# CristianSimion5/vk-raytracing-engine

Hardware: AMD Instinct MI355X
Metric: Mrays/s (higher is better)
Workload: dtype f32

## Files before the change

### vk-raytracing-engine_amd/csrc/rgen.h

```cpp
#pragma once
#include "device_math.h"
#include "device_scene.h"
#include "shade.h"

struct LaneState
{
  Payload prd;
  f3 curWeight, hitValue, hitValues;
  f3 camOrigin;
  uint32_t px;
  uint32_t lrow;
  int smpl;
  int stage;
};

VKRT_DEV uint32_t globalRow(const TraceParams& P, uint32_t lrow)
{
  if(P.stripRows == 0u)
    return lrow;
  const uint32_t s = lrow / P.stripRows, r = lrow % P.stripRows;
  return (s * P.shardCount + P.shardIndex) * P.stripRows + r;
}

VKRT_DEV bool pixelOfWork(const TraceParams& P, unsigned w, unsigned tileFirst, uint32_t& x, uint32_t& y, uint32_t& lrow)
{
  if(w >= P.tileCount * 64u)
    return false;
  const unsigned tile = tileFirst + (w >> 6), inTile = w & 63u;
  x = (tile % P.tilesX) * 8u + (inTile & 7u);
  lrow = (tile / P.tilesX) * 8u + (inTile >> 3);
  if(x >= P.fullW || lrow >= P.localRows)
    return false;
  y = globalRow(P, lrow);
  return y < P.fullH;
}
VKRT_DEV unsigned pixelSlot(const TraceParams& P, uint32_t x, uint32_t lrow)
{
  return (((lrow >> 3) * P.tilesX + (x >> 3)) << 6) | ((lrow & 7u) << 3) | (x & 7u);
}

VKRT_DEV uint32_t pixelSeed(const TraceParams& P, uint32_t x, uint32_t y)
{
  const uint32_t index = (P.flags & 1u) ? (y * P.fullW + x) : (y * x + x);
  return tea(index, P.seed);
}

VKRT_DEV f3 cameraOrigin(const TraceParams& P)
{
  float origin[4];
  mat4MulVec4(P.viewInverse, 0.0f, 0.0f, 0.0f, 1.0f, origin);
  return mk3(origin[0], origin[1], origin[2]);
}

VKRT_DEV void startSample(const TraceParams& P, LaneState& L)
{
  const float r1 = rnd(L.prd.seed);
  const float r2 = rnd(L.prd.seed);
  const float jx = P.pc.frame == 0 ? 0.5f : r1, jy = P.pc.frame == 0 ? 0.5f : r2;
  const float pcx = (float)L.px + jx, pcy = (float)globalRow(P, L.lrow) + jy;
  const float inU = pcx / (float)P.fullW, inV = pcy / (float)P.fullH;
  const float dx = inU * 2.0f - 1.0f, dy = inV * 2.0f - 1.0f;
  float target[4], direction[4];
  mat4MulVec4(P.projInverse, dx, dy, 1.0f, 1.0f, target);
  const f3 tn = normalize3(mk3(target[0], target[1], target[2]));
  mat4MulVec4(P.viewInverse, tn.x, tn.y, tn.z, 0.0f, direction);
  L.prd.hitValue = mk3(0.0f);
  L.prd.rayOrigin = L.camOrigin;
  L.prd.rayDirection = mk3(direction[0], direction[1], direction[2]);
  L.prd.depth = 0;
  L.prd.weight = mk3(0.0f);
  L.curWeight = mk3(1.0f);
  L.hitValue = mk3(0.0f);
  L.stage = 0;
}

VKRT_DEV void bindPixel(const TraceParams& P, LaneState& L, uint32_t x, uint32_t lrow)
{
  L.px = x; L.lrow = lrow;
  L.prd.isSpecular = false;
  L.prd.lightDist = 0.0f;
  L.prd.shadowRayDir = mk3(0.0f);
  L.camOrigin = cameraOrigin(P);
}

VKRT_DEV void startPixel(const TraceParams& P, LaneState& L, uint32_t x, uint32_t y, uint32_t lrow)
{
  bindPixel(P, L, x, lrow);
  L.prd.seed = pixelSeed(P, x, y);
  L.hitValues = mk3(0.0f);
  L.smpl = 0;
  startSample(P, L);
}

VKRT_DEV void storePixel(const TraceParams& P, const LaneState& L)
{
  const f3 res = L.hitValues / (float)P.pc.samples;
  float4* dst = (float4*)P.image + ((size_t)L.lrow * P.fullW + L.px);
  if(P.pc.frame > 0 && !(P.flags & VKRT_FLAG_STORE_STAGED))
  {
    const float a = 1.0f / (float)(P.pc.frame + 1);
    const float4 old = *dst;
    const f3 m = glsl_mix(mk3(old.x, old.y, old.z), res, a);
    *dst = make_float4(m.x, m.y, m.z, 1.0f);
  }
  else
    *dst = make_float4(res.x, res.y, res.z, 1.0f);
}

VKRT_DEV void blendPixel(float4* dst, float4 staged, int frame)
{
  if(frame > 0)
  {
    const float a = 1.0f / (float)(frame + 1);
    const float4 old = *dst;
    const f3 m = glsl_mix(mk3(old.x, old.y, old.z), mk3(staged.x, staged.y, staged.z), a);
    *dst = make_float4(m.x, m.y, m.z, 1.0f);
  }
  else
    *dst = make_float4(staged.x, staged.y, staged.z, 1.0f);
}

VKRT_DEV bool afterClosestRay(const TraceParams& P, LaneState& L, const RayHit& hit, const uint4 ts, f3 rayDir, ShadeStats& st)
{
  if(hit.slot >= 0)
    closestHitShader(P.sc, P.pc, hit, ts, rayDir, L.prd, st);
  else
    missShader(P.pc, L.prd);
  if(!L.prd.isSpecular && L.prd.depth != 100u)
  {
    L.stage = 1;
    return true;
  }
  return false;
}

VKRT_DEV void segmentTerms(const Payload& prd, f3 curWeight, f3& contrib, f3& nextWeight)
{
  const f3 q = prd.hitValue * curWeight;
  contrib = mk3(glsl_min(q.x, 10.0f), glsl_min(q.y, 10.0f), glsl_min(q.z, 10.0f));
  nextWeight = curWeight * prd.weight;
}

enum SegmentStep
{
  SEG_PIXEL_DONE = 0,
  SEG_CONTINUE = 1,
  SEG_SAMPLE_END = 2
};
VKRT_DEV SegmentStep stepSegment(const TraceParams& P, LaneState& L, bool shadowHit, f3 contrib, f3 nextWeight)
{
  L.stage = 0;
  if(!shadowHit)
    L.hitValue = L.hitValue + contrib;
  L.curWeight = nextWeight;
  L.prd.depth++;
  if(L.prd.depth < (uint32_t)P.pc.depth)
    return SEG_CONTINUE;
  L.hitValues = L.hitValues + L.hitValue;
  L.smpl++;
  if(L.smpl < P.pc.samples)
    return SEG_SAMPLE_END;
  storePixel(P, L);
  return SEG_PIXEL_DONE;
}

VKRT_DEV bool advanceSegment(const TraceParams& P, LaneState& L, bool shadowHit, f3 contrib, f3 nextWeight)
{
  const SegmentStep step = stepSegment(P, L, shadowHit, contrib, nextWeight);
  if(step == SEG_SAMPLE_END)
    startSample(P, L);
  return step != SEG_PIXEL_DONE;
}

VKRT_DEV bool accumulateAndAdvance(const TraceParams& P, LaneState& L, bool shadowHit)
{
  f3 contrib, nextWeight;
  segmentTerms(L.prd, L.curWeight, contrib, nextWeight);
  return advanceSegment(P, L, shadowHit, contrib, nextWeight);
}
```

### vk-raytracing-engine_amd/csrc/shade.h

```cpp
#pragma once
#include "device_math.h"
#include "device_scene.h"
#include "texel.h"
#include "traverse.h"

struct Payload
{
  f3 hitValue;
  uint32_t seed;
  uint32_t depth;
  f3 rayOrigin, rayDirection, weight;
  bool isSpecular;
  float lightDist;
  f3 shadowRayDir;
};

struct ShadeStats
{
  unsigned hits, diffuse, taps;
  const float* lut;
};

VKRT_DEV const float* ldsTexelLut(const DevScene& sc, float* lds512)
{
// ... 61 lines not shown
  st.taps++;
  f4 r;
  if(sc.textureCount == 0u || texIndex < 0 || texIndex >= (int)sc.textureCount)
  {
    r.x = r.y = r.z = r.w = 1.0f;
    return r;
  }
  DevTexture tx = sc.textures[texIndex];
  const uint32_t levels = tx.srgb >> 8;
  if(!g.on || levels <= 1u)
    return sampleTexLevel(sc, tx, nullptr, 0u, u, v, st.lut);
  const uint32_t* levelOffsets = sc.texMips + (size_t)texIndex * VKRT_MAX_MIPS;
  const float fw = (float)tx.width, fh = (float)tx.height;
  const float mxu = g.dudx * fw, mxv = g.dvdx * fh, myu = g.dudy * fw, myv = g.dvdy * fh;
  const float rx2 = mxu * mxu + mxv * mxv, ry2 = myu * myu + myv * myv;
  const bool majorX = rx2 >= ry2;
  const float rmax = sqrtf(majorX ? rx2 : ry2), rmin = sqrtf(majorX ? ry2 : rx2);
  float eta = 1.0f;
  if(rmin > 0.0f)
    eta = glsl_min(rmax / rmin, 4.0f);
  else if(rmax > 0.0f)
    eta = 4.0f;
  if(!(eta >= 1.0f))
    eta = 1.0f;
  const int N = (int)ceilf(eta);
  const float scale = rmax / eta;
  float lambda = 0.0f;
  if(scale > 1.0f && scale < 3.0e38f)
    lambda = lodLog2(scale);
  else if(!(scale <= 1.0f))
    lambda = (float)(levels - 1u);
  lambda = glsl_clamp(lambda, 0.0f, (float)(levels - 1u));
  const float fl = floorf(lambda), delta = lambda - fl;
  const uint32_t hi = (uint32_t)fl, lo = hi + 1u < levels ? hi + 1u : levels - 1u;
  const float du = majorX ? g.dudx : g.dudy, dv = majorX ? g.dvdx : g.dvdy;
  r.x = r.y = r.z = r.w = 0.0f;
  for(int i = 1; i <= N; i++)
  {
    const float o = (float)i / (float)(N + 1) - 0.5f;
    float tu = u + o * du, tv = v + o * dv;
    if(!(fabsf(tu) < 1.0e9f) || !(fabsf(tv) < 1.0e9f))
    {
      tu = u;
      tv = v;
    }
    const f4 a = sampleTexLevel(sc, tx, levelOffsets, hi, tu, tv, st.lut), b = sampleTexLevel(sc, tx, levelOffsets, lo, tu, tv, st.lut);
    r.x = r.x + (a.x * (1.0f - delta) + b.x * delta);
    r.y = r.y + (a.y * (1.0f - delta) + b.y * delta);
    r.z = r.z + (a.z * (1.0f - delta) + b.z * delta);
    r.w = r.w + (a.w * (1.0f - delta) + b.w * delta);
  }
  const float inv = 1.0f / (float)N;
  r.x = r.x * inv; r.y = r.y * inv; r.z = r.z * inv; r.w = r.w * inv;
  return r;
}

VKRT_DEV f3 pbrGetBaseColor(const DevScene& sc, const GltfPBRMaterial& mat, float tu, float tv, const TexGrad& g, ShadeStats& st)
{
  f3 color = mk3(mat.pbrBaseColorFactor[0], mat.pbrBaseColorFactor[1], mat.pbrBaseColorFactor[2]);
  if(mat.pbrBaseColorTexture > -1)
  {
    const f4 t = sampleTex(sc, mat.pbrBaseColorTexture, tu, tv, g, st);
    color = color * mk3(t.x, t.y, t.z);
  }
  return color;
}
VKRT_DEV void pbrGetMetallicRoughness(const DevScene& sc, const GltfPBRMaterial& mat, float tu, float tv, const TexGrad& g,
                                      float& metallic, float& roughness, ShadeStats& st)
{
  metallic = mat.metallicFactor;
  roughness = mat.roughnessFactor;
  if(mat.metallicRoughnessTexture > -1)
  {
    const f4 t = sampleTex(sc, mat.metallicRoughnessTexture, tu, tv, g, st);
    roughness *= t.y;
    metallic *= t.z;
  }
}
VKRT_DEV float getNDF_GGXTR(f3 N, f3 H, float alpha)
{
  float a2 = alpha * alpha;
  float NH = dot3(N, H);
  if(NH <= 0.0f)
    return 0.0f;
  float NH2 = NH * NH;
  float d = NH2 * (a2 - 1.0f) + 1.0f;
  return a2 * VKRT_INV_PI / (d * d + 1e-4f);
}
VKRT_DEV float getG_SchlickGGX(float NV, float k) { return NV / (NV * (1.0f - k) + k); }
VKRT_DEV float getG_Smith(f3 N, f3 V, f3 L, float k)
{
  float NV = fabsf(dot3(N, V));
  float NL = fabsf(dot3(N, L));
  return getG_SchlickGGX(NV, k) * getG_SchlickGGX(NL, k);
}
VKRT_DEV f3 getF_Schlick(f3 H, f3 V, f3 F0)
{
  return F0 + (mk3(1.0f) - F0) * vk_pow5(1.0f - fabsf(dot3(H, V)));
}
VKRT_DEV f3 getSpecularBRDF_Cook_Torrance(f3 N, f3 H, f3 V, f3 L, f3 F0, float roughness)
{
  float alpha = roughness * roughness;
  float k = (roughness + 1.0f) * (roughness + 1.0f) / 8.0f;
  float D = getNDF_GGXTR(N, H, alpha);
  float G = getG_Smith(N, V, L, k);
  f3 F = getF_Schlick(H, V, F0);
  float down = 4.0f * fabsf(dot3(V, N)) * fabsf(dot3(L, N)) + 1e-4f;
  return D * F * G / down;
}
VKRT_DEV f3 getSpecularBRDF_over_pdf_Cook_Torrance(f3 N, f3 H, f3 V, f3 L, f3 F0, float roughness, float ratio)
{
  float k = (roughness + 1.0f) * (roughness + 1.0f) / 8.0f;
  float pdf = (1.0f - ratio) * dot3(N, H) / (4.0f * dot3(L, H) + 1e-4f);
  float G = getG_Smith(N, V, L, k);
  f3 F = getF_Schlick(H, V, F0);
  float down = 4.0f * fabsf(dot3(V, N)) * fabsf(dot3(L, N)) + 1e-4f;
  return (F * G / down) / pdf;
}
VKRT_DEV f3 computePBR_BRDF(f3 N, f3 V, f3 L, f3 H, f3 baseColor, float metalness, float roughness)
{
  f3 F0 = mk3(0.04f);
  F0 = glsl_mix(F0, baseColor, metalness);
  f3 F = getF_Schlick(H, V, F0);
  f3 f_cook_torrance = getSpecularBRDF_Cook_Torrance(N, H, V, L, F0, roughness);
  f3 kD = mk3(1.0f) - F;
  kD = kD * (1.0f - metalness);
  f3 f_lambert = baseColor * VKRT_INV_PI;
  f3 diffuse = kD * f_lambert;
  return diffuse + f_cook_torrance;
}
VKRT_DEV f3 directLight(const GltfLight& light, f3 P, f3 N, f3 V, f3 baseColor, float metalness, float roughness, unsigned retap,
                        f3& Li, float& cosTheta, ShadeStats& st)
{
  Li = mk3(0.0f);
  cosTheta = 0.0f;
  if(light.type == 0)
  {
    f3 Ldir = mk3(light.position[0], light.position[1], light.position[2]) - P;
    float d = length3(Ldir);
    f3 L = Ldir / d;
    f3 H = normalize3(L + V);
    float attenuation = d * d;
    Li = mk3(light.color[0], light.color[1], light.color[2]) * light.intensity / attenuation;
    cosTheta = glsl_max(dot3(L, N), 0.0f);
    if(cosTheta > 0.0f)
    {
      st.taps += retap;
      return computePBR_BRDF(N, V, L, H, baseColor, metalness, roughness);
    }
  }
  return mk3(0.0f);
}

VKRT_DEV f3 xformPoint(const DevInstance& in, f3 p)
{
  f3 r;
  r.x = ((in.o2w[0] * p.x + in.o2w[1] * p.y) + in.o2w[2] * p.z) + in.o2w[3];
  r.y = ((in.o2w[4] * p.x + in.o2w[5] * p.y) + in.o2w[6] * p.z) + in.o2w[7];
  r.z = ((in.o2w[8] * p.x + in.o2w[9] * p.y) + in.o2w[10] * p.z) + in.o2w[11];
  return r;
}
VKRT_DEV f3 xformNormal(const DevInstance& in, f3 n)
{
  f3 r;
  r.x = (n.x * in.w2o[0] + n.y * in.w2o[3]) + n.z * in.w2o[6];
  r.y = (n.x * in.w2o[1] + n.y * in.w2o[4]) + n.z * in.w2o[7];
  r.z = (n.x * in.w2o[2] + n.y * in.w2o[5]) + n.z * in.w2o[8];
  return r;
}

struct HitMid
{
  f3 worldPos, N, tangent, binormal, V, baseColor, emittance;
  float metalU, roughU;
  unsigned retap;
};

VKRT_DEV void closestHitFront(const DevScene& sc, const RayHit& hit, const uint32_t instId, const uint4 ts, f3 worldRayDir, const Payload& prd,
                              ShadeStats& st, HitMid& mid)
{
  st.hits++;
  const uint32_t i0 = ts.x, i1 = ts.y, i2 = ts.z, matIndex = ts.w;
  const f3 b = mk3(1.0f - hit.u - hit.v, hit.u, hit.v);

  const BufView vPN = bufView(sc.vertexPN), vMat = bufView(sc.shadeMaterials), vInst = bufView(sc.instances);
  const float4 a0 = bufLoad4(vPN, VKRT_VERTEX_BYTES * i0), b0 = bufLoad4(vPN, VKRT_VERTEX_BYTES * i0 + 16u), tq0 = bufLoad4(vPN, VKRT_VERTEX_BYTES * i0 + 32u);
  const float4 a1 = bufLoad4(vPN, VKRT_VERTEX_BYTES * i1), b1 = bufLoad4(vPN, VKRT_VERTEX_BYTES * i1 + 16u), tq1 = bufLoad4(vPN, VKRT_VERTEX_BYTES * i1 + 32u);
  const float4 a2 = bufLoad4(vPN, VKRT_VERTEX_BYTES * i2), b2 = bufLoad4(vPN, VKRT_VERTEX_BYTES * i2 + 16u), tq2 = bufLoad4(vPN, VKRT_VERTEX_BYTES * i2 + 32u);
  const uint32_t mo = 64u * matIndex;
  const float4 m0 = bufLoad4(vMat, mo), m1 = bufLoad4(vMat, mo + 16u), ref01 = bufLoad4(vMat, mo + 32u), ref23 = bufLoad4(vMat, mo + 48u);
  const uint32_t dimB = __float_as_uint(ref01.x), baseB = __float_as_uint(ref01.y), dimM = __float_as_uint(ref01.z), baseM = __float_as_uint(ref01.w);
  const uint32_t dimN = __float_as_uint(ref23.x), baseN = __float_as_uint(ref23.y), dimE = __float_as_uint(ref23.z), baseE = __float_as_uint(ref23.w);
  DevInstance in;
  {
    const uint32_t io = 96u * instId;
    const float4 q0 = bufLoad4(vInst, io), q1 = bufLoad4(vInst, io + 16u), q2 = bufLoad4(vInst, io + 32u), q3 = bufLoad4(vInst, io + 48u), q4 = bufLoad4(vInst, io + 64u),
                 q5 = bufLoad4(vInst, io + 80u);
    in.o2w[0] = q0.x; in.o2w[1] = q0.y; in.o2w[2] = q0.z; in.o2w[3] = q0.w; in.o2w[4] = q1.x; in.o2w[5] = q1.y; in.o2w[6] = q1.z; in.o2w[7] = q1.w;
    in.o2w[8] = q2.x; in.o2w[9] = q2.y; in.o2w[10] = q2.z; in.o2w[11] = q2.w;
    in.w2o[0] = q3.x; in.w2o[1] = q3.y; in.w2o[2] = q3.z; in.w2o[3] = q3.w; in.w2o[4] = q4.x; in.w2o[5] = q4.y; in.w2o[6] = q4.z; in.w2o[7] = q4.w;
    in.w2o[8] = q5.x; in.primMesh = __float_as_int(q5.y); in.vis = 0u; in.pad = 0;
  }
  GltfPBRMaterial mat;
  mat.pbrBaseColorFactor[0] = m0.x; mat.pbrBaseColorFactor[1] = m0.y; mat.pbrBaseColorFactor[2] = m0.z; mat.pbrBaseColorFactor[3] = 1.0f;
  mat.metallicFactor = m0.w; mat.roughnessFactor = m1.x;
  mat.emissiveFactor[0] = m1.y; mat.emissiveFactor[1] = m1.z; mat.emissiveFactor[2] = m1.w;
  mat.pbrBaseColorTexture = (dimB & 0x8000u) ? 0 : -1; mat.metallicRoughnessTexture = (dimM & 0x8000u) ? 0 : -1;
  mat.normalTexture = (dimN & 0x8000u) ? 0 : -1; mat.emissiveTexture = (dimE & 0x8000u) ? 0 : -1;
  const float tu = (b0.z * b.x + b1.z * b.y) + b2.z * b.z;
  const float tv = (b0.w * b.x + b1.w * b.y) + b2.w * b.z;

  const bool emits = prd.depth == 0 || prd.isSpecular;
  const bool wantE = emits && mat.emissiveTexture > -1, wantN = mat.normalTexture > -1;
  const bool wantB = mat.pbrBaseColorTexture > -1, wantM = mat.metallicRoughnessTexture > -1;
  st.taps += (wantE ? 1u : 0u) + (wantN ? 1u : 0u) + (wantB ? 1u : 0u) + (wantM ? 1u : 0u);
  TexTap tE, tN, tB, tM;
  uint32_t e00 = 0u, e10 = 0u, e01 = 0u, e11 = 0u, n00 = 0u, n10 = 0u, n01 = 0u, n11 = 0u;
  uint32_t c00 = 0u, c10 = 0u, c01 = 0u, c11 = 0u, r00 = 0u, r10 = 0u, r01 = 0u, r11 = 0u;
  const bool pool = sc.texQuads != nullptr;
  const BufView gather = bufView(pool ? (const void*)sc.texQuads : (const void*)sc.texels);
#define VKRT_TAP(dim, base, want, tap, a, b, c, d)                                                                                     \
  if(__ballot(want) != 0ull)                                                                                                           \
  {                                                                                                                                    \
    const uint32_t w_ = ((dim) & 0x7fffu) + 1u, h_ = (((dim) >> 16) & 0x7fffu) + 1u;                                                   \
    const bool live_ = (want) && ((dim) >> 31) != 0u;                                                                                  \
    int x0_, y0_;                                                                                                                      \
    texFootprintOrigin(w_, h_, ((base) >> 31) != 0u, ((dim) >> 31) != 0u, tu, tv, tap, x0_, y0_);                                      \
    if(pool)                                                                                                                           \
    {                                                                                                                                  \
      const uint32_t rec_ = live_ ? ((uint32_t)y0_ * w_ + (uint32_t)x0_) + ((base) & 0x7fffffffu) : 0u;                                 \
      const float4 v_ = bufLoad4(gather, 16u * rec_);                                                                                  \
      a = __float_as_uint(v_.x); b = __float_as_uint(v_.y); c = __float_as_uint(v_.z); d = __float_as_uint(v_.w);                      \
    }                                                                                                                                  \
    else                                                                                                                               \
    {                                                                                                                                  \
      texFootprintTexels((base) & 0x7fffffffu, w_, h_, live_, x0_, y0_, tap);                                                          \
      a = bufLoad1(gather, 4u * tap.i00); b = bufLoad1(gather, 4u * tap.i10);                                                          \
      c = bufLoad1(gather, 4u * tap.i01); d = bufLoad1(gather, 4u * tap.i11);                                                          \
    }                                                                                                                                  \
  }
  VKRT_TAP(dimE, baseE, wantE, tE, e00, e10, e01, e11)
  VKRT_TAP(dimN, baseN, wantN, tN, n00, n10, n01, n11)
  VKRT_TAP(dimB, baseB, wantB, tB, c00, c10, c01, c11)
  VKRT_TAP(dimM, baseM, wantM, tM, r00, r10, r01, r11)
#undef VKRT_TAP

  const f3 pos = mk3(a0.x, a0.y, a0.z) * b.x + mk3(a1.x, a1.y, a1.z) * b.y + mk3(a2.x, a2.y, a2.z) * b.z;
  const f3 worldPos = xformPoint(in, pos);
  const f3 nrm = normalize3(mk3(a0.w, b0.x, b0.y) * b.x + mk3(a1.w, b1.x, b1.y) * b.y + mk3(a2.w, b2.x, b2.y) * b.z);
  const f3 worldNrm = normalize3(xformNormal(in, nrm));
  const f3 tag = normalize3(mk3(tq0.x, tq0.y, tq0.z) * b.x + mk3(tq1.x, tq1.y, tq1.z) * b.y + mk3(tq2.x, tq2.y, tq2.z) * b.z);
  f3 worldTag = normalize3(xformNormal(in, tag));
  worldTag = normalize3(worldTag - dot3(worldTag, worldNrm) * worldNrm);
  const f3 worldBin = tq0.w * cross3(worldNrm, worldTag);

  f3 emittance = mk3(0.0f);
  if(emits)
  {
    emittance = mk3(mat.emissiveFactor[0], mat.emissiveFactor[1], mat.emissiveFactor[2]);
    if(wantE)
    {
      const f4 t = texBlend(st.lut, tE, e00, e10, e01, e11);
      emittance = emittance * mk3(t.x, t.y, t.z);
    }
  }
  f3 tangent = worldTag, binormal = worldBin;
  f3 texNormal = worldNrm;
  if(wantN)
  {
    const f4 t = texBlend(st.lut, tN, n00, n10, n01, n11);
    texNormal = normalize3(mk3(t.x, t.y, t.z) * 2.0f - mk3(1.0f));
    texNormal = normalize3(tangent * texNormal.x + binormal * texNormal.y + worldNrm * texNormal.z);
    createCoordinateSystem(texNormal, tangent, binormal);
  }
  f3 baseColor = mk3(mat.pbrBaseColorFactor[0], mat.pbrBaseColorFactor[1], mat.pbrBaseColorFactor[2]);
  if(wantB)
  {
    const f4 t = texBlend(st.lut, tB, c00, c10, c01, c11);
    baseColor = baseColor * mk3(t.x, t.y, t.z);
  }
  float metalness = mat.metallicFactor, roughness = mat.roughnessFactor;
  if(wantM)
  {
    const f4 t = texBlend(st.lut, tM, r00, r10, r01, r11);
    roughness *= t.y;
    metalness *= t.z;
  }

  mid.worldPos = worldPos; mid.N = texNormal; mid.tangent = tangent; mid.binormal = binormal;
  mid.V = normalize3(-worldRayDir);
  mid.baseColor = baseColor; mid.emittance = emittance;
  mid.metalU = metalness; mid.roughU = roughness;
  mid.retap = (mat.pbrBaseColorTexture > -1 ? 1u : 0u) + (mat.metallicRoughnessTexture > -1 ? 1u : 0u);
}

VKRT_DEV bool closestHitLobe(const HitMid& mid, Payload& prd)
{
  const float ratio = 0.5f * (1.0f - mid.metalU);
  const float r1 = rnd(prd.seed);
  return r1 < ratio;
}

VKRT_DEV void closestHitTail(const DevScene& sc, const PushConstantRay& pc, const HitMid& mid, const bool diffuse, Payload& prd, ShadeStats& st)
{
  const f3 worldPos = mid.worldPos, texNormal = mid.N, tangent = mid.tangent, binormal = mid.binormal, V = mid.V, N = mid.N;
  const f3 baseColor = mid.baseColor;
  f3 emittance = mid.emittance;
  const float metalU = mid.metalU, roughU = mid.roughU;
  const unsigned retap = mid.retap;
  const float ratio = 0.5f * (1.0f - metalU);
  const float roughness = glsl_clamp(roughU, 0.01f, 0.99f);
  const float metalness = glsl_clamp(metalU, 0.01f, 0.99f);
  const f3 rayOrigin = worldPos;
  f3 rayDirection;
  float pdf;
  f3 BRDF;
  if(diffuse)
  {
    st.diffuse++;
    prd.isSpecular = false;
    const int random_index = (int)(rnd(prd.seed) * (float)pc.lightsCount);
    const float4* lq = (const float4*)&sc.lights[random_index];
    const float4 l0 = lq[0], l1 = lq[1];
    GltfLight light;
    light.position[0] = l0.x; light.position[1] = l0.y; light.position[2] = l0.z;
    light.color[0] = l0.w; light.color[1] = l1.x; light.color[2] = l1.y;
    light.intensity = l1.z; light.type = __float_as_int(l1.w);
    const f3 lightDir = mk3(light.position[0], light.position[1], light.position[2]) - worldPos;
    const float lightDistance = length3(lightDir);
    const f3 L = normalize3(lightDir);
    prd.lightDist = lightDistance;
    prd.shadowRayDir = L;
    if(dot3(L, texNormal) <= 0)
      emittance = emittance + mk3(0.0f);
    else
    {
      f3 Li;
      float cosTheta;
      const f3 brdf = directLight(light, worldPos, texNormal, V, baseColor, metalU, roughU, retap, Li, cosTheta, st);
      emittance = emittance + (float)pc.lightsCount * brdf * Li * cosTheta;
    }
    rayDirection = normalize3(samplingHemisphere(prd.seed, tangent, binormal, texNormal));
    pdf = ratio * dot3(rayDirection, texNormal) * VKRT_INV_PI;
    BRDF = (1.0f - metalness) * baseColor * VKRT_INV_PI;
  }
  else
  {
    prd.isSpecular = true;
    const float alpha = roughness * roughness;
    const f3 h = samplingNDF_GGXTR(prd.seed, alpha * alpha);
    const f3 H = normalize3(tangent * h.x + binormal * h.y + texNormal * h.z);
    const f3 L = normalize3(glsl_reflect(-V, H));
    rayDirection = L;
    f3 F0 = mk3(0.04f);
    F0 = glsl_mix(F0, baseColor, metalness);
    pdf = 1.0f;
    BRDF = getSpecularBRDF_over_pdf_Cook_Torrance(N, H, V, L, F0, roughness, ratio);
  }
  const float cosTheta = dot3(rayDirection, texNormal);
  prd.rayOrigin = rayOrigin;
  prd.rayDirection = rayDirection;
  prd.hitValue = emittance;
  prd.weight = BRDF * cosTheta / pdf;
}

VKRT_DEV void closestHitShaderInst(const DevScene& sc, const PushConstantRay& pc, const RayHit& hit, const uint32_t instId, const uint4 ts,
                                   f3 worldRayDir, Payload& prd, ShadeStats& st)
{
  HitMid mid;
  closestHitFront(sc, hit, instId, ts, worldRayDir, prd, st, mid);
  const bool diffuse = closestHitLobe(mid, prd);
  closestHitTail(sc, pc, mid, diffuse, prd, st);
}

VKRT_DEV void closestHitShader(const DevScene& sc, const PushConstantRay& pc, const RayHit& hit, const uint4 ts, f3 worldRayDir, Payload& prd,
                               ShadeStats& st)
{
  const uint32_t instId = (uint32_t)__float_as_int(sc.tris[hit.slot * VKRT_TRI_QUADS + 2].z);
  closestHitShaderInst(sc, pc, hit, instId, ts, worldRayDir, prd, st);
}
VKRT_DEV void closestHitShader(const DevScene& sc, const PushConstantRay& pc, const RayHit& hit, f3 worldRayDir, Payload& prd, ShadeStats& st)
{
  closestHitShader(sc, pc, hit, sc.triShade[hit.slot], worldRayDir, prd, st);
}

VKRT_DEV void missShader(const PushConstantRay& pc, Payload& prd)
{
  if(prd.depth == 0)
    prd.hitValue = mk3(pc.clearColor[0], pc.clearColor[1], pc.clearColor[2]) * 0.8f;
  else
    prd.hitValue = mk3(0.01f);
  prd.depth = 100;
}

VKRT_DEV void mat4MulVec4(const float* M, float v0, float v1, float v2, float v3, float* out)
{
#pragma unroll
  for(int i = 0; i < 4; i++)
    out[i] = ((M[0 + i] * v0 + M[4 + i] * v1) + M[8 + i] * v2) + M[12 + i] * v3;
}
```

### vk-raytracing-engine_amd/csrc/wavefront.hip

```cpp
#include <hip/hip_runtime.h>
#include <algorithm>
#include <cstdlib>
#include <cstring>

#include "device_math.h"
#include "device_scene.h"
#include "kernels.h"
#include "rgen.h"
#include "hybrid_gi.h"
#include "shade.h"
#include "traverse.h"
#include "traverse_wide.h"
#include "traverse_share.h"

#define WF_BLOCK 256
#define VKRT_FLAG_COUNT_WORK 2u

#include "wf_streams.h"

VKRT_DEV unsigned packFlags(const LaneState& L)
{
  return (L.prd.depth & 0xffu) | (((unsigned)L.smpl & 0xffffu) << 8) | ((L.prd.isSpecular ? 1u : 0u) << 25);
}

VKRT_DEV void loadCommon(const TraceParams& P, const WfBuffers& B, int parity, int type, unsigned i, LaneState& L)
{
  const float4 s0 = wfLoad(rec(B, parity, type, WF_S0, i)), s1 = wfLoad(rec(B, parity, type, WF_S1, i)), s2 = wfLoad(rec(B, parity, type, WF_S2, i));
  const unsigned flags = __float_as_uint(s1.w), pix = __float_as_uint(s2.w);
  L.curWeight = mk3(s0.x, s0.y, s0.z); L.prd.seed = __float_as_uint(s0.w);
  L.hitValue = mk3(s1.x, s1.y, s1.z);
  L.prd.depth = flags & 0xffu; L.smpl = (int)((flags >> 8) & 0xffffu);
  L.prd.isSpecular = ((flags >> 25) & 1u) != 0u;
  L.hitValues = mk3(s2.x, s2.y, s2.z);
  L.px = pix & 0xffffu; L.lrow = pix >> 16;
  L.camOrigin = cameraOrigin(P);
  L.prd.lightDist = 0.0f;
  L.prd.shadowRayDir = mk3(0.0f);
  L.prd.hitValue = mk3(0.0f);
  L.prd.weight = mk3(0.0f);
  L.stage = 0;
}

VKRT_DEV void storeState(const WfBuffers& B, int parity, int type, unsigned i, const LaneState& L, f3 weight)
{
  wfStore(rec(B, parity, type, WF_S0, i), make_float4(weight.x, weight.y, weight.z, __uint_as_float(L.prd.seed)));
  wfStore(rec(B, parity, type, WF_S1, i), make_float4(L.hitValue.x, L.hitValue.y, L.hitValue.z, __uint_as_float(packFlags(L))));
  wfStore(rec(B, parity, type, WF_S2, i), make_float4(L.hitValues.x, L.hitValues.y, L.hitValues.z, __uint_as_float(L.px | (L.lrow << 16))));
}

VKRT_DEV void storeClosest(const WfBuffers& B, int parity, unsigned i, const LaneState& L)
{
  wfStore(rec(B, parity, WF_C, WF_R0, i), make_float4(L.prd.rayOrigin.x, L.prd.rayOrigin.y, L.prd.rayOrigin.z, 10000.0f));
  wfStore(rec(B, parity, WF_C, WF_R1, i), make_float4(L.prd.rayDirection.x, L.prd.rayDirection.y, L.prd.rayDirection.z, 0.0f));
  storeState(B, parity, WF_C, i, L, L.curWeight);
}

VKRT_DEV void storeShadow(const WfBuffers& B, int parity, int type, unsigned i, const LaneState& L, f3 contrib, f3 nextWeight)
{
  wfStore(rec(B, parity, type, WF_R0, i), make_float4(L.prd.rayOrigin.x, L.prd.rayOrigin.y, L.prd.rayOrigin.z, L.prd.lightDist - 0.1f));
  wfStore(rec(B, parity, type, WF_R1, i), make_float4(L.prd.shadowRayDir.x, L.prd.shadowRayDir.y, L.prd.shadowRayDir.z, L.prd.lightDist));
  if(type == WF_P)
    wfStore(rec(B, parity, type, WF_R2, i), make_float4(L.prd.rayDirection.x, L.prd.rayDirection.y, L.prd.rayDirection.z, 0.0f));
  storeState(B, parity, type, i, L, nextWeight);
  wfStore(rec(B, parity, type, WF_S3, i), make_float4(contrib.x, contrib.y, contrib.z, 0.0f));
}

VKRT_DEV int finishSegment(const TraceParams& P, const WfBuffers& B, LaneState& L, bool shadowHit, f3 contrib, f3 nextWeight)
{
  const SegmentStep step = stepSegment(P, L, shadowHit, contrib, nextWeight);
  if(step == SEG_SAMPLE_END)
  {
    if(P.flags & VKRT_FLAG_SAMPLE_SYNC)
    {
      wfStore(B.sampleState + pixelSlot(P, L.px, L.lrow), make_float4(L.hitValues.x, L.hitValues.y, L.hitValues.z, __uint_as_float(L.prd.seed)));
      return -1;
    }
    startSample(P, L);
  }
  return step == SEG_PIXEL_DONE ? -1 : WF_C;
}

VKRT_DEV unsigned claimSlots(const WfBuffers& B, int parity, int to, unsigned lane, unsigned* wsum)
{
  const unsigned wave = threadIdx.x >> 6, nw = blockDim.x >> 6;
  const unsigned long long m[WF_TYPES] = {__ballot(to == WF_C), __ballot(to == WF_S), __ballot(to == WF_P)};
  if(lane == 0)
  {
#pragma unroll
    for(int t = 0; t < WF_TYPES; t++) wsum[t * (nw + 1) + wave] = (unsigned)__popcll(m[t]);
  }
  __syncthreads();
  if(threadIdx.x < WF_TYPES)
  {
    unsigned* w = wsum + threadIdx.x * (nw + 1);
    unsigned tot = 0;
    for(unsigned k = 0; k < nw; k++)
    {
      const unsigned c = w[k];
      w[k] = tot;
      tot += c;
    }
    w[nw] = tot ? atomicAdd(countOf(B, parity, (int)threadIdx.x), tot) : 0u;
  }
  __syncthreads();
  if(to < 0)
    return 0u;
  const unsigned long long below = (1ull << lane) - 1ull;
  const unsigned long long mine = to == WF_C ? m[0] : to == WF_S ? m[1] : m[2];
  return wsum[to * (nw + 1) + nw] + wsum[to * (nw + 1) + wave] + (unsigned)__popcll(mine & below);
}

__global__ __launch_bounds__(WF_BLOCK) void k_wf_init(const TraceParams P, const WfBuffers B)
{
  const unsigned lane = lane_id();
  const unsigned w = blockIdx.x * blockDim.x + threadIdx.x;
  bool alive = false;
  unsigned nPixels = 0;
  LaneState L;
  uint32_t x, y, lrow;
  if(pixelOfWork(P, w, P.tileFirst, x, y, lrow))
  {
    startPixel(P, L, x, y, lrow);
    nPixels = 1;
    if(P.pc.samples <= 0 || P.pc.depth <= 0)
      storePixel(P, L);
    else
      alive = true;
  }
  __shared__ unsigned wsum[WF_TYPES * (WF_BLOCK / 64 + 1)];
  const unsigned slot = claimSlots(B, 0, alive ? WF_C : -1, lane, wsum);
  if(alive)
    storeClosest(B, 0, slot, L);
  __shared__ unsigned long long red[VKRT_COUNTER_STRIDE * (WF_BLOCK / 64)];
  const unsigned vals[6] = {0, 0, 0, 0, 0, nPixels};
  blockAddCounters(&P.counters->v[blockIdx.x % VKRT_COUNTER_SLOTS][0], vals, 6, red);
}

__global__ __launch_bounds__(WF_BLOCK) void k_wf_sample_init(const TraceParams P, const WfBuffers B, const int round, const int smpl)
{
  const unsigned lane = lane_id();
  const unsigned w = blockIdx.x * blockDim.x + threadIdx.x;
  bool alive = false;
  LaneState L;
  uint32_t x, y, lrow;
  if(pixelOfWork(P, w, P.tileFirst, x, y, lrow))
  {
    const float4 st = wfLoad(B.sampleState + pixelSlot(P, x, lrow));
    bindPixel(P, L, x, lrow);
    L.prd.seed = __float_as_uint(st.w);
    L.hitValues = mk3(st.x, st.y, st.z);
    L.smpl = smpl;
    startSample(P, L);
    alive = true;
  }
  __shared__ unsigned wsum[WF_TYPES * (WF_BLOCK / 64 + 1)];
  const unsigned slot = claimSlots(B, round & 1, alive ? WF_C : -1, lane, wsum);
  if(alive)
    storeClosest(B, round & 1, slot, L);
}

VKRT_DEV bool advanceSegmentHybrid(const TraceParams& P, const HybridGi& G, LaneState& L, bool shadowHit, f3 contrib, f3 nextWeight, float lightDist)
{
  L.stage = 0;
  if(giSegmentStep(P.pc, L.prd, L.curWeight, L.hitValue, L.hitValues.x, shadowHit, contrib, nextWeight, lightDist))
    return true;
  hybridStorePixel(P, G, (size_t)L.lrow * P.fullW + L.px, true, L.hitValue, L.hitValues.x, L.hitValues.y);
  return false;
}

struct ShadeLds
{
  float lut[512];
  unsigned wsum[WF_TYPES * (WF_BLOCK / 64 + 1)];
};

VKRT_DEV bool pixelOfWave(const TraceParams& P, unsigned w, unsigned tileFirst, uint32_t& x, uint32_t& y, uint32_t& lrow)
{
  if(w >= P.tileCount * 64u)
    return false;
  const unsigned tile = (unsigned)__builtin_amdgcn_readfirstlane((int)(tileFirst + (w >> 6))), inTile = w & 63u;
  x = (tile % P.tilesX) * 8u + (inTile & 7u);
  lrow = (tile / P.tilesX) * 8u + (inTile >> 3);
  if(x >= P.fullW || lrow >= P.localRows)
    return false;
  y = globalRow(P, lrow);
  return y < P.fullH;
}

template <bool PAIR, bool HYBRID, bool CAMERA = false>
VKRT_DEV void shadeHitBlock(const TraceParams& P, const WfBuffers& B, const HybridGi& G, const int par, const unsigned count, const unsigned block, ShadeLds& lds,
                            const int smpl = 0)
{
  const int type = PAIR ? WF_P : WF_C;
  const unsigned lane = lane_id();
  const unsigned qi = block * WF_BLOCK + threadIdx.x;
  ShadeStats st = shadeStatsInit<WF_BLOCK>(P.sc, lds.lut);
  unsigned* wsum = lds.wsum;
  int to = -1;
  LaneState L;
  f3 contrib = mk3(0.0f), nextWeight = mk3(0.0f);
  uint32_t x = 0, y = 0, lrow = 0;
  if(CAMERA ? pixelOfWave(P, qi, P.tileFirst, x, y, lrow) : qi < count)
  {
    if(CAMERA)
    {
      bindPixel(P, L, x, lrow);
      if(smpl == 0)
      {
        L.prd.seed = pixelSeed(P, x, y);
        L.hitValues = mk3(0.0f);
      }
      else
      {
        const float4 s = wfLoad(B.sampleState + (P.tileFirst * 64u + qi));
        L.prd.seed = __float_as_uint(s.w);
        L.hitValues = mk3(s.x, s.y, s.z);
      }
      L.smpl = smpl;
      startSample(P, L);
    }
    else
      loadCommon(P, B, par, type, qi, L);
    const float4 h = wfLoad(rec(B, par, type, WF_H0, qi)), t4 = wfLoad(rec(B, par, type, WF_H1, qi));
    if(!CAMERA)
    {
      const float4 rd = wfLoad(rec(B, par, type, PAIR ? WF_R2 : WF_R1, qi));
      L.prd.rayDirection = mk3(rd.x, rd.y, rd.z);
    }
    L.prd.rayOrigin = mk3(0.0f);
    if(PAIR)
    {
      const float4 s3 = wfLoad(rec(B, par, WF_P, WF_S3, qi));
      const bool shadowHit = __float_as_int(h.x) != 0;
      if(HYBRID)
        (void)advanceSegmentHybrid(P, G, L, shadowHit, mk3(s3.x, s3.y, s3.z), L.curWeight, L.prd.depth == 1u ? wfLoad(rec(B, par, WF_P, WF_R1, qi)).w : 0.0f);
      else
        (void)advanceSegment(P, L, shadowHit, mk3(s3.x, s3.y, s3.z), L.curWeight);
    }
    RayHit hit;
    hit.t = h.x; hit.u = h.y; hit.v = h.z; hit.slot = __float_as_int(h.w);
    const uint4 ts = make_uint4(__float_as_uint(t4.x), __float_as_uint(t4.y), __float_as_uint(t4.z), __float_as_uint(t4.w));
    if(hit.slot >= 0)
      closestHitShaderInst(P.sc, P.pc, hit, (uint32_t)hit.slot, ts, L.prd.rayDirection, L.prd, st);
    else
      missShader(P.pc, L.prd);
    segmentTerms(L.prd, L.curWeight, contrib, nextWeight);
    const bool dead = !HYBRID && (P.flags & VKRT_FLAG_SKIP_DEAD_SHADOW) != 0u && contrib.x == 0.0f && contrib.y == 0.0f && contrib.z == 0.0f;
    if(!L.prd.isSpecular && L.prd.depth != 100u && !dead)
      to = (L.prd.depth + 1u < (uint32_t)P.pc.depth) ? WF_P : WF_S;
    else if(HYBRID)
      to = advanceSegmentHybrid(P, G, L, false, contrib, nextWeight, 0.0f) ? WF_C : -1;
    else
      to = finishSegment(P, B, L, false, contrib, nextWeight);
  }
  const unsigned slot = claimSlots(B, par ^ 1, to, lane, wsum);
  if(to == WF_C)
    storeClosest(B, par ^ 1, slot, L);
  else if(to == WF_P)
    storeShadow(B, par ^ 1, WF_P, slot, L, contrib, nextWeight);
  else if(to == WF_S)
    storeShadow(B, par ^ 1, WF_S, slot, L, contrib, nextWeight);
  if(P.flags & VKRT_FLAG_COUNT_WORK)
  {
    __shared__ unsigned long long red[VKRT_COUNTER_STRIDE * (WF_BLOCK / 64)];
    const unsigned vals[5] = {0, 0, st.hits, st.diffuse, st.taps};
    blockAddCounters(&P.counters->v[blockIdx.x % VKRT_COUNTER_SLOTS][0], vals, 5, red);
  }
}

template <bool HYBRID>
VKRT_DEV void shadeShadowBlock(const TraceParams& P, const WfBuffers& B, const HybridGi& G, const int par, const unsigned count, const unsigned block, ShadeLds& lds)
{
  const unsigned lane = lane_id();
  const unsigned qi = block * WF_BLOCK + threadIdx.x;
  unsigned* wsum = lds.wsum;
  bool toClosest = false;
  LaneState L;
  if(qi < count)
  {
    loadCommon(P, B, par, WF_S, qi, L);
    const float4 h = wfLoad(rec(B, par, WF_S, WF_H0, qi)), s3 = wfLoad(rec(B, par, WF_S, WF_S3, qi));
    L.prd.rayOrigin = mk3(0.0f);
    L.prd.rayDirection = mk3(0.0f);
    const bool shadowHit = __float_as_int(h.w) >= 0;
    if(HYBRID)
      toClosest = advanceSegmentHybrid(P, G, L, shadowHit, mk3(s3.x, s3.y, s3.z), L.curWeight, L.prd.depth == 1u ? wfLoad(rec(B, par, WF_S, WF_R1, qi)).w : 0.0f);
    else
      toClosest = finishSegment(P, B, L, shadowHit, mk3(s3.x, s3.y, s3.z), L.curWeight) == WF_C;
  }
  const unsigned slot = claimSlots(B, par ^ 1, toClosest ? WF_C : -1, lane, wsum);
  if(toClosest)
    storeClosest(B, par ^ 1, slot, L);
}

#if defined(__HIP_DEVICE_COMPILE__)
#define WF_SCALAR_FP32 __attribute__((target("no-packed-fp32-ops")))
#else
#define WF_SCALAR_FP32
#endif
template <bool HYBRID>
VKRT_DEV void shadeRound(const TraceParams& P, const WfBuffers& B, const HybridGi& G, const int round)
{
  const int par = round & 1;
  const unsigned cC = *countOf(B, par, WF_C), cS = *countOf(B, par, WF_S), cP = *countOf(B, par, WF_P);
  const unsigned nC = (cC + WF_BLOCK - 1) / WF_BLOCK, nP = (cP + WF_BLOCK - 1) / WF_BLOCK, nS = (cS + WF_BLOCK - 1) / WF_BLOCK;
  unsigned blk = blockIdx.x;
  __shared__ ShadeLds lds;
  if(blk < nC)
    shadeHitBlock<false, HYBRID>(P, B, G, par, cC, blk, lds);
  else if((blk -= nC) < nP)
    shadeHitBlock<true, HYBRID>(P, B, G, par, cP, blk, lds);
  else if((blk -= nP) < nS)
    shadeShadowBlock<HYBRID>(P, B, G, par, cS, blk, lds);
}
WF_SCALAR_FP32 __global__ __launch_bounds__(WF_BLOCK) void k_wf_shade(const TraceParams P, const WfBuffers B, const int round)
{
  const HybridGi none{};
  shadeRound<false>(P, B, none, round);
}
WF_SCALAR_FP32 __global__ __launch_bounds__(WF_BLOCK) void k_wf_shade_hybrid(const TraceParams P, const WfBuffers B, const HybridGi G, const int round)
{
  shadeRound<true>(P, B, G, round);
}
WF_SCALAR_FP32 __global__ __launch_bounds__(WF_BLOCK) void k_wf_shade_camera(const TraceParams P, const WfBuffers B, const int round, const int smpl)
{
  const HybridGi none{};
  __shared__ ShadeLds lds;
  shadeHitBlock<false, false, true>(P, B, none, round & 1, 0u, blockIdx.x, lds, smpl);
}

__global__ __launch_bounds__(WF_BLOCK) void k_hy_gi_init(const TraceParams P, const WfBuffers B, const HybridGi G, const uint2* tmp)
{
  const unsigned lane = lane_id();
  const unsigned w = blockIdx.x * blockDim.x + threadIdx.x;
  bool alive = false;
  LaneState L;
  uint32_t x, y, lrow;
  if(pixelOfWork(P, w, P.tileFirst, x, y, lrow))
  {
    const size_t p = (size_t)lrow * P.fullW + x;
    const GbufferPixel g = loadGbufferPixel(G, p);
    const uint2 t = tmp[p];
    const float alpha = __uint_as_float(t.y);
    if(g.shaded)
    {
      bindPixel(P, L, x, lrow);
      L.prd.seed = t.x;
      giFirstRay(P, g, L.prd, L.curWeight);
      L.hitValue = mk3(0.0f);
      L.hitValues = mk3(0.0f, alpha, 0.0f);
      L.smpl = 0;
      L.stage = 0;
      alive = L.prd.depth < (uint32_t)P.pc.depth;
    }
    if(!alive)
      hybridStorePixel(P, G, p, g.shaded, mk3(0.0f), 0.0f, alpha);
  }
  __shared__ unsigned wsum[WF_TYPES * (WF_BLOCK / 64 + 1)];
  const unsigned slot = claimSlots(B, 0, alive ? WF_C : -1, lane, wsum);
  if(alive)
    storeClosest(B, 0, slot, L);
}

__global__ __launch_bounds__(WF_BLOCK) void k_wf_blend(const TraceParams P, const float4* stage)
{
  uint32_t x, y, lrow;
  if(pixelOfWork(P, blockIdx.x * blockDim.x + threadIdx.x, P.tileFirst, x, y, lrow))
  {
    const size_t p = (size_t)lrow * P.fullW + x;
    blendPixel((float4*)P.image + p, stage[p], P.pc.frame);
  }
}

#define WF_CTRL_BYTES (256 * VKRT_WF_MAX_LANES)
size_t vkrt_wf_state_bytes(uint32_t pathCapacity, int groups)
{
  const size_t g = (size_t)std::max(groups, 1);
  return g * pathCapacity * 2 * WF_SLOTS * sizeof(float4) + (g > 1 ? g * pathCapacity * sizeof(float4) : 0) + g * pathCapacity * sizeof(float4) +
         WF_CTRL_BYTES;
}

void vkrt_wf_carve(void* base, uint32_t pathCapacity, int groups, WfBuffers* B)
{
  const size_t g = (size_t)std::max(groups, 1);
  char* p = (char*)base;
  B->ctrl = (unsigned*)p;
  p += WF_CTRL_BYTES;
  B->planes = (float4*)p;
  p += g * pathCapacity * 2 * WF_SLOTS * sizeof(float4);
  B->stage = g > 1 ? (float4*)p : nullptr;
  p += g > 1 ? g * pathCapacity * sizeof(float4) : 0;
  B->sampleState = (float4*)p;
  B->capacity = pathCapacity;
  B->groups = (uint32_t)g;
}

static unsigned pixelBlocks(const TraceParams& P) { return (P.tileCount * 64u + WF_BLOCK - 1) / WF_BLOCK; }
static hipError_t subframeBegin(const TraceParams& P, const WfBuffers& B, bool init, hipStream_t stream)
{
  const hipError_t e = hipMemsetAsync(B.ctrl, 0, 64, stream);
  if(e == hipSuccess && init)
    hipLaunchKernelGGL(k_wf_init, dim3(pixelBlocks(P)), dim3(WF_BLOCK), 0, stream, P, B);
  return e;
}
static void launchTraverse(const TraceParams& P, const WfBuffers& B, int r, unsigned travBlock, bool count, hipStream_t stream)
{
  const unsigned work = P.tileCount * 64u, tb = (travBlock == 256u || travBlock == 128u) ? travBlock : 64u;
  vkrt_wf_launch_traverse(P, B, r, tb, count, dim3(2 * ((work + tb - 1) / tb) + 4), (size_t)P.sc.stackCap * tb * sizeof(int), stream);
}
static void subframeRound(const TraceParams& P, const WfBuffers& B, int r, int cameraSample, unsigned travBlock, bool count, hipStream_t stream, WfTiming* timing)
{
  const bool timed = timing && timing->events && 2 * (timing->used + 1) <= timing->capacity;
  if(timed)
    (void)hipEventRecord(timing->events[2 * timing->used], stream);
  if(cameraSample >= 0)
    vkrt_wf_launch_traverse_camera(P, B, r, cameraSample, count, (size_t)P.sc.stackCap * 64u * sizeof(int), stream);
  else
    launchTraverse(P, B, r, travBlock, count, stream);
  if(timed)
  {
    (void)hipEventRecord(timing->events[2 * timing->used + 1], stream);
    timing->used++;
  }
  if(cameraSample >= 0)
    hipLaunchKernelGGL(k_wf_shade_camera, dim3(pixelBlocks(P)), dim3(WF_BLOCK), 0, stream, P, B, r, cameraSample);
  else
    hipLaunchKernelGGL(k_wf_shade, dim3(pixelBlocks(P) + 3), dim3(WF_BLOCK), 0, stream, P, B, r);
}

hipError_t vkrt_launch_wavefront(const TraceParams& P, const WfBuffers& B, const WfOptions& opt, int frames, uint32_t seedStep, bool count,
                                 hipStream_t stream, WfTiming* timing, const WfAsync* async)
{
  const WfCall call{P.pc.samples, P.pc.depth, (P.flags & VKRT_FLAG_SAMPLE_SYNC) != 0u, (P.flags & VKRT_FLAG_CAMERA_ROUNDS) != 0u, P.tileCount, frames,
                    opt.inFlight, opt.subframes, (int)B.groups, async ? async->count : 0, timing != nullptr};
  const WfLanes lanes = wfLanes(call);
  const int L = lanes.F * lanes.S;
  const bool staged = lanes.F > 1;
  if(staged && wfPoolEvents(lanes.frames) > async->poolSize)
    return hipErrorInvalidValue;
  hipStream_t laneStream[VKRT_WF_MAX_LANES];
  WfBuffers Bq[VKRT_WF_MAX_LANES];
  laneStream[0] = stream;
  Bq[0] = B;
  const size_t groupQuads = (size_t)2 * WF_SLOTS * B.capacity;
  for(int q = 0; L > 1 && q < L; q++)
  {
    const int g = q / lanes.S, j = q % lanes.S;
    const uint32_t tile0 = lanes.tileFirst(j);
    Bq[q].ctrl = B.ctrl + 64 * q;
    Bq[q].planes = B.planes + (size_t)g * groupQuads + (size_t)2 * WF_SLOTS * ((size_t)tile0 * 64u);
    Bq[q].stage = staged ? B.stage + (size_t)g * B.capacity : nullptr;
    Bq[q].sampleState = B.sampleState + (size_t)g * B.capacity;
    Bq[q].capacity = (lanes.tileFirst(j + 1) - tile0) * 64u;
    Bq[q].groups = 1;
    laneStream[q] = async->streams[q];
  }
  int forked = 0;
  auto joinLanes = [&]() {
    hipError_t first = hipSuccess;
    for(int q = 0; q < forked; q++)
    {
      hipError_t x = hipEventRecord(async->join[q], laneStream[q]);
      if(x == hipSuccess) x = hipStreamWaitEvent(stream, async->join[q], 0);
      if(x != hipSuccess)
      {
        (void)hipStreamSynchronize(laneStream[q]);
        if(first == hipSuccess) first = x;
      }
    }
    return first;
  };
  hipError_t e = hipSuccess;
  if(L > 1 && (e = hipEventRecord(async->fork, stream)) != hipSuccess) return e;
  for(int q = 0; L > 1 && q < L; q++)
  {
    if((e = hipStreamWaitEvent(laneStream[q], async->fork, 0)) != hipSuccess)
    {
// ... 72 lines not shown
```

Measured before the change: 5892.

## Cut register pressure in wavefront shade kernels and target five waves per EU

Removes the cached camera origin from the per-lane state and recomputes it where needed. The instance transform load is deferred until after the texture taps, with asm barriers to pin the interpolation sums, so fewer values stay live across the taps. Loading of the accumulated sample sums is delayed until after shading in the non-hybrid path, and the inner shadow step no longer runs the full sample-end and store logic. The shade kernels are annotated with waves_per_eu(5) to steer register allocation toward higher occupancy, at the risk of spills or more reloads.

```diff
diff --git a/vk-raytracing-engine_amd/csrc/rgen.h b/vk-raytracing-engine_amd/csrc/rgen.h
--- a/vk-raytracing-engine_amd/csrc/rgen.h
+++ b/vk-raytracing-engine_amd/csrc/rgen.h
@@ -7,7 +7,6 @@
 {
   Payload prd;
   f3 curWeight, hitValue, hitValues;
-  f3 camOrigin;
   uint32_t px;
   uint32_t lrow;
   int smpl;
@@ -65,7 +64,7 @@
   const f3 tn = normalize3(mk3(target[0], target[1], target[2]));
   mat4MulVec4(P.viewInverse, tn.x, tn.y, tn.z, 0.0f, direction);
   L.prd.hitValue = mk3(0.0f);
-  L.prd.rayOrigin = L.camOrigin;
+  L.prd.rayOrigin = cameraOrigin(P);
   L.prd.rayDirection = mk3(direction[0], direction[1], direction[2]);
   L.prd.depth = 0;
   L.prd.weight = mk3(0.0f);
@@ -80,7 +79,6 @@
   L.prd.isSpecular = false;
   L.prd.lightDist = 0.0f;
   L.prd.shadowRayDir = mk3(0.0f);
-  L.camOrigin = cameraOrigin(P);
 }
 
 VKRT_DEV void startPixel(const TraceParams& P, LaneState& L, uint32_t x, uint32_t y, uint32_t lrow)
@@ -164,6 +162,15 @@
   return SEG_PIXEL_DONE;
 }
 
+VKRT_DEV void stepInnerSegment(LaneState& L, bool shadowHit, f3 contrib, f3 nextWeight)
+{
+  L.stage = 0;
+  if(!shadowHit)
+    L.hitValue = L.hitValue + contrib;
+  L.curWeight = nextWeight;
+  L.prd.depth++;
+}
+
 VKRT_DEV bool advanceSegment(const TraceParams& P, LaneState& L, bool shadowHit, f3 contrib, f3 nextWeight)
 {
   const SegmentStep step = stepSegment(P, L, shadowHit, contrib, nextWeight);
diff --git a/vk-raytracing-engine_amd/csrc/shade.h b/vk-raytracing-engine_amd/csrc/shade.h
--- a/vk-raytracing-engine_amd/csrc/shade.h
+++ b/vk-raytracing-engine_amd/csrc/shade.h
@@ -237,6 +237,9 @@
   return mk3(0.0f);
 }
 
+VKRT_DEV void settle(float& x) { asm volatile("" : "+v"(x)); }
+VKRT_DEV void settle(f3& v) { settle(v.x); settle(v.y); settle(v.z); }
+
 VKRT_DEV f3 xformPoint(const DevInstance& in, f3 p)
 {
   f3 r;
@@ -276,16 +279,6 @@
   const float4 m0 = bufLoad4(vMat, mo), m1 = bufLoad4(vMat, mo + 16u), ref01 = bufLoad4(vMat, mo + 32u), ref23 = bufLoad4(vMat, mo + 48u);
   const uint32_t dimB = __float_as_uint(ref01.x), baseB = __float_as_uint(ref01.y), dimM = __float_as_uint(ref01.z), baseM = __float_as_uint(ref01.w);
   const uint32_t dimN = __float_as_uint(ref23.x), baseN = __float_as_uint(ref23.y), dimE = __float_as_uint(ref23.z), baseE = __float_as_uint(ref23.w);
-  DevInstance in;
-  {
-    const uint32_t io = 96u * instId;
-    const float4 q0 = bufLoad4(vInst, io), q1 = bufLoad4(vInst, io + 16u), q2 = bufLoad4(vInst, io + 32u), q3 = bufLoad4(vInst, io + 48u), q4 = bufLoad4(vInst, io + 64u),
-                 q5 = bufLoad4(vInst, io + 80u);
-    in.o2w[0] = q0.x; in.o2w[1] = q0.y; in.o2w[2] = q0.z; in.o2w[3] = q0.w; in.o2w[4] = q1.x; in.o2w[5] = q1.y; in.o2w[6] = q1.z; in.o2w[7] = q1.w;
-    in.o2w[8] = q2.x; in.o2w[9] = q2.y; in.o2w[10] = q2.z; in.o2w[11] = q2.w;
-    in.w2o[0] = q3.x; in.w2o[1] = q3.y; in.w2o[2] = q3.z; in.w2o[3] = q3.w; in.w2o[4] = q4.x; in.w2o[5] = q4.y; in.w2o[6] = q4.z; in.w2o[7] = q4.w;
-    in.w2o[8] = q5.x; in.primMesh = __float_as_int(q5.y); in.vis = 0u; in.pad = 0;
-  }
   GltfPBRMaterial mat;
   mat.pbrBaseColorFactor[0] = m0.x; mat.pbrBaseColorFactor[1] = m0.y; mat.pbrBaseColorFactor[2] = m0.z; mat.pbrBaseColorFactor[3] = 1.0f;
   mat.metallicFactor = m0.w; mat.roughnessFactor = m1.x;
@@ -294,6 +287,11 @@
   mat.normalTexture = (dimN & 0x8000u) ? 0 : -1; mat.emissiveTexture = (dimE & 0x8000u) ? 0 : -1;
   const float tu = (b0.z * b.x + b1.z * b.y) + b2.z * b.z;
   const float tv = (b0.w * b.x + b1.w * b.y) + b2.w * b.z;
+
+  f3 pos = mk3(a0.x, a0.y, a0.z) * b.x + mk3(a1.x, a1.y, a1.z) * b.y + mk3(a2.x, a2.y, a2.z) * b.z;
+  f3 nrmSum = mk3(a0.w, b0.x, b0.y) * b.x + mk3(a1.w, b1.x, b1.y) * b.y + mk3(a2.w, b2.x, b2.y) * b.z;
+  f3 tagSum = mk3(tq0.x, tq0.y, tq0.z) * b.x + mk3(tq1.x, tq1.y, tq1.z) * b.y + mk3(tq2.x, tq2.y, tq2.z) * b.z;
+  settle(pos); settle(nrmSum); settle(tagSum);
 
   const bool emits = prd.depth == 0 || prd.isSpecular;
   const bool wantE = emits && mat.emissiveTexture > -1, wantN = mat.normalTexture > -1;
@@ -330,14 +328,25 @@
   VKRT_TAP(dimM, baseM, wantM, tM, r00, r10, r01, r11)
 #undef VKRT_TAP
 
-  const f3 pos = mk3(a0.x, a0.y, a0.z) * b.x + mk3(a1.x, a1.y, a1.z) * b.y + mk3(a2.x, a2.y, a2.z) * b.z;
-  const f3 worldPos = xformPoint(in, pos);
-  const f3 nrm = normalize3(mk3(a0.w, b0.x, b0.y) * b.x + mk3(a1.w, b1.x, b1.y) * b.y + mk3(a2.w, b2.x, b2.y) * b.z);
-  const f3 worldNrm = normalize3(xformNormal(in, nrm));
-  const f3 tag = normalize3(mk3(tq0.x, tq0.y, tq0.z) * b.x + mk3(tq1.x, tq1.y, tq1.z) * b.y + mk3(tq2.x, tq2.y, tq2.z) * b.z);
+  DevInstance in;
+  {
+    uint32_t io = 96u * instId;
+    asm volatile("" : "+v"(io));
+    const float4 q0 = bufLoad4(vInst, io), q1 = bufLoad4(vInst, io + 16u), q2 = bufLoad4(vInst, io + 32u), q3 = bufLoad4(vInst, io + 48u), q4 = bufLoad4(vInst, io + 64u),
+                 q5 = bufLoad4(vInst, io + 80u);
+    in.o2w[0] = q0.x; in.o2w[1] = q0.y; in.o2w[2] = q0.z; in.o2w[3] = q0.w; in.o2w[4] = q1.x; in.o2w[5] = q1.y; in.o2w[6] = q1.z; in.o2w[7] = q1.w;
+    in.o2w[8] = q2.x; in.o2w[9] = q2.y; in.o2w[10] = q2.z; in.o2w[11] = q2.w;
+    in.w2o[0] = q3.x; in.w2o[1] = q3.y; in.w2o[2] = q3.z; in.w2o[3] = q3.w; in.w2o[4] = q4.x; in.w2o[5] = q4.y; in.w2o[6] = q4.z; in.w2o[7] = q4.w;
+    in.w2o[8] = q5.x; in.primMesh = __float_as_int(q5.y); in.vis = 0u; in.pad = 0;
+  }
+  f3 worldPos = xformPoint(in, pos);
+  const f3 nrm = normalize3(nrmSum);
+  f3 worldNrm = normalize3(xformNormal(in, nrm));
+  const f3 tag = normalize3(tagSum);
   f3 worldTag = normalize3(xformNormal(in, tag));
   worldTag = normalize3(worldTag - dot3(worldTag, worldNrm) * worldNrm);
-  const f3 worldBin = tq0.w * cross3(worldNrm, worldTag);
+  f3 worldBin = tq0.w * cross3(worldNrm, worldTag);
+  settle(worldPos); settle(worldNrm); settle(worldTag); settle(worldBin);
 
   f3 emittance = mk3(0.0f);
   if(emits)
diff --git a/vk-raytracing-engine_amd/csrc/wavefront.hip b/vk-raytracing-engine_amd/csrc/wavefront.hip
--- a/vk-raytracing-engine_amd/csrc/wavefront.hip
+++ b/vk-raytracing-engine_amd/csrc/wavefront.hip
@@ -23,17 +23,24 @@
   return (L.prd.depth & 0xffu) | (((unsigned)L.smpl & 0xffffu) << 8) | ((L.prd.isSpecular ? 1u : 0u) << 25);
 }
 
-VKRT_DEV void loadCommon(const TraceParams& P, const WfBuffers& B, int parity, int type, unsigned i, LaneState& L)
-{
-  const float4 s0 = wfLoad(rec(B, parity, type, WF_S0, i)), s1 = wfLoad(rec(B, parity, type, WF_S1, i)), s2 = wfLoad(rec(B, parity, type, WF_S2, i));
-  const unsigned flags = __float_as_uint(s1.w), pix = __float_as_uint(s2.w);
+VKRT_DEV void loadSums(const WfBuffers& B, int parity, int type, unsigned i, LaneState& L)
+{
+  const float4 s2 = wfLoad(rec(B, parity, type, WF_S2, i));
+  const unsigned pix = __float_as_uint(s2.w);
+  L.hitValues = mk3(s2.x, s2.y, s2.z);
+  L.px = pix & 0xffffu; L.lrow = pix >> 16;
+}
+
+VKRT_DEV void loadCommon(const TraceParams& P, const WfBuffers& B, int parity, int type, unsigned i, LaneState& L, bool sums = true)
+{
+  const float4 s0 = wfLoad(rec(B, parity, type, WF_S0, i)), s1 = wfLoad(rec(B, parity, type, WF_S1, i));
+  const unsigned flags = __float_as_uint(s1.w);
   L.curWeight = mk3(s0.x, s0.y, s0.z); L.prd.seed = __float_as_uint(s0.w);
   L.hitValue = mk3(s1.x, s1.y, s1.z);
   L.prd.depth = flags & 0xffu; L.smpl = (int)((flags >> 8) & 0xffffu);
   L.prd.isSpecular = ((flags >> 25) & 1u) != 0u;
-  L.hitValues = mk3(s2.x, s2.y, s2.z);
-  L.px = pix & 0xffffu; L.lrow = pix >> 16;
-  L.camOrigin = cameraOrigin(P);
+  if(sums)
+    loadSums(B, parity, type, i, L);
   L.prd.lightDist = 0.0f;
   L.prd.shadowRayDir = mk3(0.0f);
   L.prd.hitValue = mk3(0.0f);
@@ -220,7 +227,7 @@
       startSample(P, L);
     }
     else
-      loadCommon(P, B, par, type, qi, L);
+      loadCommon(P, B, par, type, qi, L, HYBRID);
     const float4 h = wfLoad(rec(B, par, type, WF_H0, qi)), t4 = wfLoad(rec(B, par, type, WF_H1, qi));
     if(!CAMERA)
     {
@@ -235,7 +242,7 @@
       if(HYBRID)
         (void)advanceSegmentHybrid(P, G, L, shadowHit, mk3(s3.x, s3.y, s3.z), L.curWeight, L.prd.depth == 1u ? wfLoad(rec(B, par, WF_P, WF_R1, qi)).w : 0.0f);
       else
-        (void)advanceSegment(P, L, shadowHit, mk3(s3.x, s3.y, s3.z), L.curWeight);
+        stepInnerSegment(L, shadowHit, mk3(s3.x, s3.y, s3.z), L.curWeight);
     }
     RayHit hit;
     hit.t = h.x; hit.u = h.y; hit.v = h.z; hit.slot = __float_as_int(h.w);
@@ -244,6 +251,8 @@
       closestHitShaderInst(P.sc, P.pc, hit, (uint32_t)hit.slot, ts, L.prd.rayDirection, L.prd, st);
     else
       missShader(P.pc, L.prd);
+    if(!CAMERA && !HYBRID)
+      loadSums(B, par, type, qi, L);
     segmentTerms(L.prd, L.curWeight, contrib, nextWeight);
     const bool dead = !HYBRID && (P.flags & VKRT_FLAG_SKIP_DEAD_SHADOW) != 0u && contrib.x == 0.0f && contrib.y == 0.0f && contrib.z == 0.0f;
     if(!L.prd.isSpecular && L.prd.depth != 100u && !dead)
@@ -298,6 +307,7 @@
 #else
 #define WF_SCALAR_FP32
 #endif
+#define WF_FIVE_WAVES __attribute__((amdgpu_waves_per_eu(5)))
 template <bool HYBRID>
 VKRT_DEV void shadeRound(const TraceParams& P, const WfBuffers& B, const HybridGi& G, const int round)
 {
@@ -313,7 +323,7 @@
   else if((blk -= nP) < nS)
     shadeShadowBlock<HYBRID>(P, B, G, par, cS, blk, lds);
 }
-WF_SCALAR_FP32 __global__ __launch_bounds__(WF_BLOCK) void k_wf_shade(const TraceParams P, const WfBuffers B, const int round)
+WF_SCALAR_FP32 WF_FIVE_WAVES __global__ __launch_bounds__(WF_BLOCK) void k_wf_shade(const TraceParams P, const WfBuffers B, const int round)
 {
   const HybridGi none{};
   shadeRound<false>(P, B, none, round);
@@ -322,7 +332,7 @@
 {
   shadeRound<true>(P, B, G, round);
 }
-WF_SCALAR_FP32 __global__ __launch_bounds__(WF_BLOCK) void k_wf_shade_camera(const TraceParams P, const WfBuffers B, const int round, const int smpl)
+WF_SCALAR_FP32 WF_FIVE_WAVES __global__ __launch_bounds__(WF_BLOCK) void k_wf_shade_camera(const TraceParams P, const WfBuffers B, const int round, const int smpl)
 {
   const HybridGi none{};
   __shared__ ShadeLds lds;
```

After: 5898 (median of 3 runs). No clear change (+0.1%).
